# NeRF-3DTalker/NeRF-3DTalker-code

Hardware: AMD Instinct MI355X
Metric: rendered frames/sec @512^2 x 64 samples/ray (higher is better)
Workload: dtype bf16; 1 GPU; cfg2-R: 16 heads/GPU/step, 64x64 rays x 64 samples -> fused MLP+composite -> neural renderer -> 512x512 RGB (+ background image); rays_per_frame=4096, samples_per_ray=64, parallelism=frames sharded over 1 rank(s), no data-path collective, ranks_seen_by_backend=1

## Files before the change

### nerf-3dtalker-code_amd/csrc/nerf_fwd_x16.hip

```cpp
#include "x16_core.h"


#ifndef X16_SAVE_DEPTH
#define X16_SAVE_DEPTH 3
#endif
template <int PREC>
struct X16SaveStage {
    unsigned char* tile0;
    unsigned* gate0;
};

#define X16_BIAS_SLOT 1536
#ifndef X16_SAVE_LDS_BIAS
#define X16_SAVE_LDS_BIAS 1
#endif
struct X16BiasLds {
    unsigned char* slots;
    unsigned addr;
    __device__ __forceinline__ void stage_in(const float* table, const int n, const int slot, const int lane) const {
#pragma unroll
        for (int i = 0; i < 6; ++i)
            if (64 * i < n)
                __builtin_amdgcn_global_load_lds((const GLOBAL_AS void*)(table + 64 * i + lane), (LDS_AS void*)(slots + slot * X16_BIAS_SLOT + 256 * i), 4, 0, 0);
    }
};

template <int PREC, int NB, int WAVES, int KS, int KPE, int NT, int MODE, bool SAVE = false, class WS>
__device__ __forceinline__ void x16_stage(WS& ws, const float* __restrict__ bias,
                                          const typename X16<PREC>::frag (&pe_reg)[NB][4], const unsigned char* pe_lds,
                                          const typename X16<PREC>::frag (&hin)[NB][24], typename X16<PREC>::frag (&hout)[NB][24],
                                          float (&aux)[NB], float* const (&po)[NB], const bool (&live)[NB], const int lane,
                                          const X16SaveStage<PREC>* sv = nullptr, const short relu_lo = 0,
                                          const unsigned bias_lds = 0 ) {
    typedef typename X16<PREC>::frag frag;
    static_assert(!SAVE || NB == 1, "the training forward runs one block per wave");
    const int h = lane >> 5, c = lane & 31;
    float red[NB][32];
    unsigned gate_word = 0;
    const frag ones = X16<PREC>::ones_frag();
    float bias_cur = 0.0f, bias_nxt = 0.0f;
    constexpr bool LB = SAVE && X16_SAVE_LDS_BIAS;
    if constexpr (LB) {
        x16_bias_read<0>(bias_cur, bias_lds);
        asm volatile("s_waitcnt lgkmcnt(0)" : "+v"(bias_cur));
    } else {
        bias_cur = bias[c];
    }
    constexpr bool PACKS = (MODE == MODE_HIDDEN || MODE == MODE_LINEAR);
    f32x16 acc[1][NB];
    auto finish_half = [&](const int t, const int half) {
#pragma unroll
        for (int nb = 0; nb < NB; ++nb) {
            float v[8];
#pragma unroll
            for (int r = 0; r < 8; ++r) v[r] = acc[0][nb][8 * half + r];
            frag f = X16<PREC>::pack(v);
            if (MODE == MODE_HIDDEN) f = X16<PREC>::relu(f, relu_lo);
            hout[nb][2 * t + half] = f;
        }
    };
    static_for<0, NT>([&](auto ot_c) {
        constexpr int ot = decltype(ot_c)::value;
        constexpr int cur = 0;
        X16_T(const unsigned long long s0 = x16_now();)
        {
            const frag bf = X16<PREC>::bias_frag(bias_cur, h == 0);
            if constexpr (LB) {
                if constexpr (ot + 1 < NT) x16_bias_read<(ot + 1) * 128>(bias_nxt, bias_lds);
            } else {
                if (ot + 1 < NT) bias_cur = bias[(ot + 1) * 32 + c];
            }
            f32x16 zero;
#pragma unroll
            for (int r = 0; r < 16; ++r) zero[r] = 0.0f;
            const f32x16 binit = X16<PREC>::mfma(bf, ones, zero);
#pragma unroll
            for (int nb = 0; nb < NB; ++nb) acc[cur][nb] = binit;
        }
        X16_T(const unsigned long long s1 = x16_now(); const unsigned long long rv0 = ws.t_rv;)
        static_for<0, KS>([&](auto ks_c) {
            constexpr int ks = decltype(ks_c)::value;
            const frag a_cur = ws.template next<MODE == MODE_COMPOSITE, NT * KS, ot * KS + ks>();
#pragma unroll
            for (int nb = 0; nb < NB; ++nb) {
                frag b;
                if (ks < KPE) {
                    if (pe_lds) b = *reinterpret_cast<const frag*>(pe_lds + (nb * 4 + ks) * X16_PIECE);
                    else b = pe_reg[nb][ks < 4 ? ks : 0];
                } else {
                    b = hin[nb][ks >= KPE ? ks - KPE : 0];
                }
                acc[cur][nb] = X16<PREC>::mfma(a_cur, b, acc[cur][nb]);
            }
        });
        if constexpr (LB && ot + 1 < NT) {
            asm volatile("" : "+v"(bias_nxt), "+v"(acc[cur][0]));
            bias_cur = bias_nxt;
        }
        X16_T(const unsigned long long s2 = x16_now();)
        if (PACKS) {
            finish_half(ot, 0);
            finish_half(ot, 1);
        }
        if constexpr (SAVE && PACKS) {
#ifndef X16_DIAG_NOIMG
            x16_image_store<PREC>(hout[0][2 * ot], hout[0][2 * ot + 1], sv->tile0 + ot * 2 * X16_PIECE);
            ws.note_stores(2);
#endif
#ifndef X16_DIAG_NOGATE
            unsigned m = 0;
#pragma unroll
            for (int half = 0; half < 2; ++half) {
                const s16x8 hv = __builtin_bit_cast(s16x8, hout[0][2 * ot + half]);
#pragma unroll
                for (int j = 0; j < 8; ++j) m |= (hv[j] != 0 ? 1u : 0u) << (8 * half + j);
            }
            if constexpr (ot & 1) {
                __builtin_nontemporal_store(gate_word | (m << 16), sv->gate0 + (ot >> 1) * 64);
                ws.note_stores(1);
            } else {
                gate_word = m;
            }
#endif
        }
#pragma unroll
        for (int nb = 0; nb < NB; ++nb) {
            if (MODE == MODE_DENSITY) {
                aux[nb] = acc[cur][nb][0];
            } else if (MODE == MODE_COMPOSITE) {
#pragma unroll
                for (int r = 0; r < 16; ++r) red[nb][(ot & 1) * 16 + r] = fmaxf(acc[cur][nb][r], 0.0f) * aux[nb];
                if constexpr (SAVE) {
#pragma unroll
                    for (int half = 0; half < 2; ++half) {
                        float v[8];
#pragma unroll
                        for (int r = 0; r < 8; ++r) v[r] = fmaxf(acc[cur][nb][8 * half + r], 0.0f);
                        __builtin_nontemporal_store(X16<PREC>::pack(v), reinterpret_cast<frag*>(sv->tile0 + (2 * ot + half) * X16_PIECE));
                    }
                    ws.note_stores(2);
                }
                if (ot & 1) {
                    float s = butterfly32(red[nb], c);
                    const int v = ((c & 1) << 4) | ((c & 2) << 2) | (c & 4) | ((c & 8) >> 2) | ((c & 16) >> 4);
                    const int reg = v & 15, tile = (ot - 1) + (v >> 4);
                    if (live[nb]) po[nb][tile * 32 + (reg & 3) + 8 * (reg >> 2) + 4 * h] = s;
                }
            }
        }
        X16_T(const unsigned long long s3 = x16_now(); ws.t_bias += s1 - s0; ws.t_mfma += (s2 - s1) - (ws.t_rv - rv0); ws.t_epi += s3 - s2;
              if (ws.tl && ws.tile_no >= 20 && ws.tile_no < 34 && (threadIdx.x & 63) == 0) {
                  ws.tl[4 + 2 * (ws.tile_no - 20)] = (float)(s1 & 0xFFFFFF);
                  ws.tl[5 + 2 * (ws.tile_no - 20)] = (float)(s2 & 0xFFFFFF);
              }
              ++ws.tile_no;)
    });
}

struct X16TrainSave {
    unsigned char* xT;
    unsigned char* gS;
    float* geo;
    unsigned* gates;
};

template <int PREC, int NB, int WAVES, bool SAVE = false>
__device__ __forceinline__ void nerf_fwd_x16_body(
    const N3dtGeom& g, const unsigned char* __restrict__ packed, const float* __restrict__ fold, const float* __restrict__ xy,
    const float* __restrict__ R, const float* __restrict__ T, const float* __restrict__ Kinv, const float* __restrict__ t_rand,
    float* __restrict__ part, float* __restrict__ wlocal, int bpr, long total_blocks, unsigned char* lds, const int wave,
    const X16TrainSave tsv = X16TrainSave{nullptr, nullptr, nullptr, nullptr}) {
    typedef typename X16<PREC>::frag frag;
    const int lane = threadIdx.x & 63;
    const int c = lane & 31, h = lane >> 5;

    typedef WeightStream<PREC, WAVES, X16_NCHUNK, X16_NBUF, SAVE ? X16_SAVE_DEPTH : X16_DEPTH> WS;
    WS ws;
    ws.gsrc = packed + (size_t)wave * WS::PPW * X16_PIECE + lane * 16;
    ws.ring = lds;
    ws.lds_addr0 = (unsigned)(size_t)(LDS_AS unsigned char*)lds + lane * 16;
    ws.wave = wave;
    ws.prologue_issue();
    unsigned char* pe_lds = lds + X16_NBUF * X16_CH * X16_PIECE + (size_t)wave * NB * 4 * X16_PIECE + lane * 16;

    bool live[NB];
    float* po[NB];
    long blk[NB];
    float dist[NB], zval[NB];
    frag pe[NB][4];
    int frame = 0;
    long ray0 = 0;
#pragma unroll
    for (int nb = 0; nb < NB; ++nb) {
        long bidx = ((long)blockIdx.x * WAVES + wave) * NB + nb;
        live[nb] = bidx < total_blocks;
        if (!live[nb]) bidx = total_blocks - 1;
        blk[nb] = bidx;
        po[nb] = part + (size_t)bidx * N3DT_PART_STRIDE;
        const int sb = (int)(bidx % bpr);
        const long rayg = bidx / bpr;
        const int ray = (int)(rayg % g.n_rays);
        const int b = (int)(rayg / g.n_rays);
        if (nb == 0) frame = b, ray0 = rayg;
        float p[3];
        n3dt_sample_point(g, xy, R, T, Kinv, t_rand, b, ray, sb * X16_BS + c, p, dist[nb], zval[nb]);
        float rh[3], rl[3];
#pragma unroll
        for (int i = 0; i < 3; ++i) {
            const float inv2pi_hi = 0.15915494f, inv2pi_lo = 6.2195e-09f;
            rh[i] = p[i] * inv2pi_hi;
            rl[i] = fmaf(p[i], inv2pi_hi, -rh[i]) + p[i] * inv2pi_lo;
        }
#pragma unroll
        for (int ks = 0; ks < 4; ++ks) {
            float v[8];
#pragma unroll
            for (int j = 0; j < 8; ++j)
                v[j] = pe_fast(p[0], p[1], p[2], rh[0], rh[1], rh[2], rl[0], rl[1], rl[2],
                               32 * (ks >> 1) + 16 * (ks & 1) + 8 * (j >> 2) + 4 * h + (j & 3));
            pe[nb][ks] = X16<PREC>::pack(v);
            *reinterpret_cast<frag*>(pe_lds + (nb * 4 + ks) * X16_PIECE) = pe[nb][ks];
        }
    }
    const float* fb = fold + (size_t)__builtin_amdgcn_readfirstlane(frame) * N3DT_FOLD_STRIDE;
    const float* b10 = fb + n3dt_bias_offset(10);
#if defined(X16_DIAG_VD_SELECT_ALL)
#if defined(X16_DIAG_VD_TERNARY)
    b10 = g.vd_dim > 0 ? fold + n3dt_rayfold_offset(g.batch) + (size_t)__builtin_amdgcn_readfirstlane((int)ray0) * N3DT_RAYFOLD_STRIDE
                       : fb + n3dt_bias_offset(10);
#elif defined(X16_DIAG_VD_NO_RFL)
    if (g.vd_dim > 0) b10 = fold + n3dt_rayfold_offset(g.batch) + (size_t)ray0 * N3DT_RAYFOLD_STRIDE;
#else
    if (g.vd_dim > 0) b10 = fold + n3dt_rayfold_offset(g.batch) + (size_t)__builtin_amdgcn_readfirstlane((int)ray0) * N3DT_RAYFOLD_STRIDE;
#endif
#else
    if constexpr (NB == 1) {
        if (g.vd_dim > 0) b10 = fold + n3dt_rayfold_offset(g.batch) + (size_t)__builtin_amdgcn_readfirstlane((int)ray0) * N3DT_RAYFOLD_STRIDE;
    }
#endif
    X16SaveStage<PREC> svs;
    unsigned char* xT_blk = nullptr;
    const long rec = live[0] ? blk[0] : total_blocks;
    if constexpr (SAVE) {
        xT_blk = tsv.xT + (size_t)rec * X16_XT_TILES * 2 * X16_PIECE + x16_image_lane_offset(lane);
        x16_image_store<PREC>(pe[0][0], pe[0][1], xT_blk);
        x16_image_store<PREC>(pe[0][2], pe[0][3], xT_blk + 2 * X16_PIECE);
    }
    auto sv_hidden = [&](const int l) -> const X16SaveStage<PREC>* {
        if constexpr (SAVE) {
            svs.tile0 = xT_blk + (size_t)(2 + 12 * l) * 2 * X16_PIECE;
            svs.gate0 = tsv.gates + ((size_t)rec * 8 + l) * 6 * 64 + lane;
            return &svs;
        } else {
            return nullptr;
        }
    };
    X16BiasLds bl;
    if constexpr (SAVE && X16_SAVE_LDS_BIAS) {
        bl.slots = lds + X16_NBUF * X16_CH * X16_PIECE + (size_t)WAVES * NB * 4 * X16_PIECE + (size_t)wave * 2 * X16_BIAS_SLOT;
        bl.addr = (unsigned)(size_t)(LDS_AS unsigned char*)bl.slots + 4 * c;
        bl.stage_in(fb + n3dt_bias_offset(0), 384, 0, lane);
    }
    auto bias_slot = [&](const int k, const int next_table, const int next_n) -> unsigned {
        if constexpr (SAVE && X16_SAVE_LDS_BIAS) {
            if (next_table >= 0) bl.stage_in(next_table == 10 ? b10 : fb + n3dt_bias_offset(next_table), next_n, (k + 1) & 1, lane);
            return bl.addr + (k & 1) * X16_BIAS_SLOT;
        } else {
            return 0u;
        }
    };
    ws.prologue_wait();
    X16_T(if (wlocal && live[0]) ws.tl = wlocal + (size_t)blk[0] * X16_BS;)

    frag ha[NB][24], hb[NB][24];
    float aux[NB];
    x16_stage<PREC, NB, WAVES, 4, 4, 12, MODE_HIDDEN, SAVE>(ws, fb + n3dt_bias_offset(0), pe, nullptr, ha, ha, aux, po, live, lane, sv_hidden(0), 0, bias_slot(0, 1, 384));
    x16_stage<PREC, NB, WAVES, 24, 0, 12, MODE_HIDDEN, SAVE>(ws, fb + n3dt_bias_offset(1), pe, nullptr, ha, hb, aux, po, live, lane, sv_hidden(1), 0, bias_slot(1, 2, 384));
    x16_stage<PREC, NB, WAVES, 24, 0, 12, MODE_HIDDEN, SAVE>(ws, fb + n3dt_bias_offset(2), pe, nullptr, hb, ha, aux, po, live, lane, sv_hidden(2), 0, bias_slot(2, 3, 384));
    x16_stage<PREC, NB, WAVES, 24, 0, 12, MODE_HIDDEN, SAVE>(ws, fb + n3dt_bias_offset(3), pe, nullptr, ha, hb, aux, po, live, lane, sv_hidden(3), 0, bias_slot(3, 4, 384));
    x16_stage<PREC, NB, WAVES, 24, 0, 12, MODE_HIDDEN, SAVE>(ws, fb + n3dt_bias_offset(4), pe, nullptr, hb, ha, aux, po, live, lane, sv_hidden(4), 0, bias_slot(4, 5, 384));
    x16_stage<PREC, NB, WAVES, 28, 4, 12, MODE_HIDDEN, SAVE>(ws, fb + n3dt_bias_offset(5), pe, pe_lds, ha, hb, aux, po, live, lane, sv_hidden(5), 0, bias_slot(5, 6, 384));
    x16_stage<PREC, NB, WAVES, 24, 0, 12, MODE_HIDDEN, SAVE>(ws, fb + n3dt_bias_offset(6), pe, nullptr, hb, ha, aux, po, live, lane, sv_hidden(6), 0, bias_slot(6, 7, 384));
    x16_stage<PREC, NB, WAVES, 24, 0, 12, MODE_HIDDEN, SAVE>(ws, fb + n3dt_bias_offset(7), pe, nullptr, ha, hb, aux, po, live, lane, sv_hidden(7), 0, bias_slot(7, 10, 192));
    x16_stage<PREC, NB, WAVES, 24, 0, 1, MODE_DENSITY, false>(ws, fb + n3dt_bias_offset(8), pe, nullptr, hb, ha, aux, po, live, lane);
#pragma unroll
    for (int nb = 0; nb < NB; ++nb) {
        float sp = __shfl(aux[nb], c, 64);
        if constexpr (SAVE) {
            if (live[nb] && h == 0) {
                tsv.geo[(size_t)blk[nb] * 64 + c] = sp;
                tsv.geo[(size_t)blk[nb] * 64 + 32 + c] = dist[nb];
            }
        }
        float sigma = fmaxf(sp, 0.0f);
#if defined(X16_DIAG_REMASK_DEAD_LANES)
        asm volatile("" : "+v"(dist[nb]), "+v"(zval[nb]));
        if ((int)(blk[nb] % bpr) * X16_BS + c >= g.n_samples) dist[nb] = 0.0f, zval[nb] = 0.0f;
#endif
        float alpha = 1.0f - expf(-sigma * dist[nb]);
        float x = 1.0f - alpha + 1e-10f;
        float Tl = n3dt_exclusive_prod<32>(x, c);
        float w = alpha * Tl;
        float s0 = w, s1 = w * zval[nb];
#pragma unroll
        for (int off = 16; off > 0; off >>= 1) {
            s0 += __shfl_xor(s0, off, 32);
            s1 += __shfl_xor(s1, off, 32);
        }
        float tprod = __shfl(Tl * x, 31, 32);
        if (live[nb] && lane == 0) {
            po[nb][N3DT_G + 0] = s0;
            po[nb][N3DT_G + 1] = s1;
            po[nb][N3DT_G + 2] = tprod;
            po[nb][N3DT_G + 3] = 0.0f;
        }
#ifndef X16_STAMP
        if (live[nb] && wlocal && h == 0) wlocal[(size_t)blk[nb] * X16_BS + c] = w;
#endif
        aux[nb] = w;
    }
    if constexpr (SAVE) {
        svs.tile0 = tsv.gS + (size_t)rec * 12 * X16_PIECE + lane * 16;
        svs.gate0 = nullptr;
    }
    x16_stage<PREC, NB, WAVES, 24, 0, 6, MODE_COMPOSITE, SAVE>(ws, b10, pe, nullptr, hb, ha, aux, po, live, lane,
                                                                     SAVE ? &svs : nullptr, 0, bias_slot(8, -1, 0));
#ifdef X16_STAMP
    if (wlocal && lane == 0 && live[0]) {
        float* dbg = wlocal + (size_t)blk[0] * X16_BS;
        dbg[0] = (float)ws.t_bias;
        dbg[1] = (float)ws.t_mfma;
        dbg[2] = (float)ws.t_epi;
        dbg[3] = (float)ws.t_rv;
    }
#endif
}

template <int PREC, int NB, int WAVES>
__global__ __launch_bounds__(WAVES * 64, 1) void nerf_fwd_x16_kernel(
    N3dtGeom g, const unsigned char* __restrict__ packed, const float* __restrict__ fold, const float* __restrict__ xy,
    const float* __restrict__ R, const float* __restrict__ T, const float* __restrict__ Kinv, const float* __restrict__ t_rand,
    float* __restrict__ part, float* __restrict__ wlocal, int bpr, long total_blocks) {
    extern __shared__ __attribute__((aligned(16))) unsigned char lds[];
    const int wave = __builtin_amdgcn_readfirstlane(threadIdx.x >> 6);
    nerf_fwd_x16_body<PREC, NB, WAVES>(g, packed, fold, xy, R, T, Kinv, t_rand, part, wlocal, bpr, total_blocks, lds, wave);
}

template <int WAVES>
__global__ __launch_bounds__(WAVES * 64, 1) void nerf_fwd_x16_train_kernel(
    N3dtGeom g, const unsigned char* __restrict__ packed, const float* __restrict__ fold, const float* __restrict__ xy,
    const float* __restrict__ R, const float* __restrict__ T, const float* __restrict__ Kinv, const float* __restrict__ t_rand,
    float* __restrict__ part, float* __restrict__ wlocal, int bpr, long total_blocks, X16TrainSave tsv) {
    extern __shared__ __attribute__((aligned(16))) unsigned char lds[];
    const int wave = __builtin_amdgcn_readfirstlane(threadIdx.x >> 6);
    nerf_fwd_x16_body<N3DT_BF16, 1, WAVES, true>(g, packed, fold, xy, R, T, Kinv, t_rand, part, wlocal, bpr, total_blocks, lds, wave,
                                                        tsv);
}

#ifndef X16_TRAIN_WAVES
#define X16_TRAIN_WAVES 8
#endif
extern "C" void n3dt_launch_nerf_fwd_x16_train(const N3dtGeom* g, const void* packed, const float* fold, const float* xy, const float* R,
                                               const float* T, const float* Kinv, const float* t_rand, float* part, float* wlocal,
                                               void* xT, void* gS, float* geo, void* gates, hipStream_t stream) {
    constexpr int WAVES = X16_TRAIN_WAVES;
    const int bpr = (g->n_samples + X16_BS - 1) / X16_BS;
    const long total = (long)g->batch * g->n_rays * bpr;
    const int grid = (int)((total + WAVES - 1) / WAVES);
    const size_t lds_bytes = X16_NBUF * X16_CH * X16_PIECE + (size_t)WAVES * 4 * X16_PIECE + (size_t)WAVES * 2 * X16_BIAS_SLOT;
    auto kern = nerf_fwd_x16_train_kernel<WAVES>;
    (void)hipFuncSetAttribute(reinterpret_cast<const void*>(kern), hipFuncAttributeMaxDynamicSharedMemorySize, (int)lds_bytes);
    X16TrainSave tsv{reinterpret_cast<unsigned char*>(xT), reinterpret_cast<unsigned char*>(gS), geo, reinterpret_cast<unsigned*>(gates)};
    hipLaunchKernelGGL(kern, dim3(grid), dim3(WAVES * 64), lds_bytes, stream, *g, reinterpret_cast<const unsigned char*>(packed), fold, xy,
                       R, T, Kinv, t_rand, part, wlocal, bpr, total, tsv);
}

template <int PREC, int NB, int WAVES>
static void launch_x16(const N3dtGeom* g, const void* packed, const float* fold, const float* xy, const float* R, const float* T,
                       const float* Kinv, const float* t_rand, float* part, float* wlocal, hipStream_t stream) {
    const int bpr = (g->n_samples + X16_BS - 1) / X16_BS;
    const long total = (long)g->batch * g->n_rays * bpr;
    const long per_wg = (long)WAVES * NB;
    const int grid = (int)((total + per_wg - 1) / per_wg);
    const size_t lds_bytes = X16_NBUF * X16_CH * X16_PIECE + (size_t)WAVES * NB * 4 * X16_PIECE;
    auto kern = nerf_fwd_x16_kernel<PREC, NB, WAVES>;
    (void)hipFuncSetAttribute(reinterpret_cast<const void*>(kern), hipFuncAttributeMaxDynamicSharedMemorySize, (int)lds_bytes);
    hipLaunchKernelGGL(kern, dim3(grid), dim3(WAVES * 64), lds_bytes, stream, *g, reinterpret_cast<const unsigned char*>(packed),
                       fold, xy, R, T, Kinv, t_rand, part, wlocal, bpr, total);
}

extern "C" void n3dt_launch_nerf_fwd_x16(const N3dtGeom* g, int precision, const void* packed, const float* fold, const float* xy,
                                         const float* R, const float* T, const float* Kinv, const float* t_rand, float* part,
                                         float* wlocal, hipStream_t stream) {
    static const int wide = [] {
        const char* e = getenv("N3DT_X16_TILING");
        const char* d = getenv("N3DT_X16_TILING2_DIAG");
        const int t = e ? atoi(e) : X16_DEFAULT_TILING;
        return (t == 2 && !(d && atoi(d) == 1)) ? 1 : t;
    }();
    const long blocks = (long)g->batch * g->n_rays * ((g->n_samples + X16_BS - 1) / X16_BS);
    const bool use_wide = wide == 2 && g->vd_dim == 0 && (((long)g->n_rays * ((g->n_samples + X16_BS - 1) / X16_BS)) % 2 == 0) && blocks >= 2;
    if (precision == N3DT_BF16) {
        if (use_wide) launch_x16<N3DT_BF16, 2, 4>(g, packed, fold, xy, R, T, Kinv, t_rand, part, wlocal, stream);
        else launch_x16<N3DT_BF16, 1, 8>(g, packed, fold, xy, R, T, Kinv, t_rand, part, wlocal, stream);
    } else {
        if (use_wide) launch_x16<N3DT_F16, 2, 4>(g, packed, fold, xy, R, T, Kinv, t_rand, part, wlocal, stream);
        else launch_x16<N3DT_F16, 1, 8>(g, packed, fold, xy, R, T, Kinv, t_rand, part, wlocal, stream);
    }
}
```

### nerf-3dtalker-code_amd/csrc/x16_core.h

```cpp
#pragma once
#include <stdlib.h>

#include <type_traits>

#include "n3dt_device.h"
#include "n3dt_layout.h"

typedef __bf16 bf16x8 __attribute__((ext_vector_type(8)));

#define X16_BS 32
#define X16_CH 24
#define X16_PIECE 1024
#define X16_NCHUNK (2280 / X16_CH)
#define X16_XT_TILES 98
#define GLOBAL_AS __attribute__((address_space(1)))
#define LDS_AS __attribute__((address_space(3)))

template <int PREC>
struct X16;
template <>
struct X16<N3DT_BF16> {
    typedef bf16x8 frag;
    static __device__ __forceinline__ f32x16 mfma(frag a, frag b, f32x16 c) {
        return __builtin_amdgcn_mfma_f32_32x32x16_bf16(a, b, c, 0, 0, 0);
    }
    static __device__ __forceinline__ f32x4 mfma16(frag a, frag b, f32x4 c) {
        return __builtin_amdgcn_mfma_f32_16x16x32_bf16(a, b, c, 0, 0, 0);
    }
    static __device__ __forceinline__ frag pack(const float* v) {
        frag f;
#pragma unroll
        for (int j = 0; j < 8; ++j) f[j] = (__bf16)v[j];
        return f;
    }
    static __device__ __forceinline__ frag relu(frag f, short lo) {
        s16x8 s = __builtin_bit_cast(s16x8, f);
        s = __builtin_elementwise_max(s, (s16x8)(lo));
        return __builtin_bit_cast(frag, s);
    }
    static __device__ __forceinline__ frag bias_frag(float b, bool lower_half) {
        __bf16 hi = (__bf16)b;
        __bf16 lo = (__bf16)(b - (float)hi);
        frag f;
#pragma unroll
        for (int j = 0; j < 8; ++j) f[j] = (__bf16)0.0f;
        if (lower_half) {
            f[0] = hi;
            f[1] = lo;
        }
        return f;
    }
    static __device__ __forceinline__ frag ones_frag() {
        frag f;
#pragma unroll
        for (int j = 0; j < 8; ++j) f[j] = (__bf16)(j < 2 ? 1.0f : 0.0f);
        return f;
    }
};
template <>
struct X16<N3DT_F16> {
    typedef f16x8 frag;
    static __device__ __forceinline__ f32x16 mfma(frag a, frag b, f32x16 c) {
        return __builtin_amdgcn_mfma_f32_32x32x16_f16(a, b, c, 0, 0, 0);
    }
    static __device__ __forceinline__ f32x4 mfma16(frag a, frag b, f32x4 c) {
        return __builtin_amdgcn_mfma_f32_16x16x32_f16(a, b, c, 0, 0, 0);
    }
    static __device__ __forceinline__ frag pack(const float* v) {
        frag f;
#pragma unroll
        for (int j = 0; j < 8; ++j) f[j] = (_Float16)v[j];
        return f;
    }
    static __device__ __forceinline__ frag relu(frag f, short lo) {
        s16x8 s = __builtin_bit_cast(s16x8, f);
        s = __builtin_elementwise_max(s, (s16x8)(lo));
        return __builtin_bit_cast(frag, s);
    }
    static __device__ __forceinline__ frag bias_frag(float b, bool lower_half) {
        _Float16 hi = (_Float16)b;
        _Float16 lo = (_Float16)(b - (float)hi);
        frag f;
#pragma unroll
        for (int j = 0; j < 8; ++j) f[j] = (_Float16)0.0f;
        if (lower_half) {
            f[0] = hi;
            f[1] = lo;
        }
        return f;
    }
    static __device__ __forceinline__ frag ones_frag() {
        frag f;
#pragma unroll
        for (int j = 0; j < 8; ++j) f[j] = (_Float16)(j < 2 ? 1.0f : 0.0f);
        return f;
    }
};

#ifndef X16_DEPTH
#define X16_DEPTH 3
#endif
#ifndef X16_DEFAULT_TILING
#define X16_DEFAULT_TILING 1
#endif
#ifndef X16_NBUF
#define X16_NBUF 3
#endif
#define X16_CHUNK_BYTES (X16_CH * X16_PIECE)

#ifdef X16_STAMP
__device__ __forceinline__ unsigned long long x16_now() {
    unsigned long long t;
    __builtin_amdgcn_sched_barrier(0);
    asm volatile("s_memtime %0\n\ts_waitcnt lgkmcnt(0)" : "=s"(t)::"memory");
    __builtin_amdgcn_sched_barrier(0);
    return t;
}
#define X16_T(x) x
#else
#define X16_T(x)
#endif

template <int I, int N, class F>
__device__ __forceinline__ void static_for(F&& f) {
    if constexpr (I < N) {
        f(std::integral_constant<int, I>{});
        static_for<I + 1, N>(f);
    }
}

template <class T>
__device__ __forceinline__ void x16_pin(T& v) {
    static_assert(sizeof(T) <= 8, "scalar register pair at most");
    asm volatile("" : "+s"(v));
}
template <class T>
__device__ __forceinline__ void x16_pin(T*& p) {
    unsigned long long v = (unsigned long long)p;
    asm volatile("" : "+s"(v));
    p = (T*)(GLOBAL_AS T*)v;
}
template <class T>
__device__ __forceinline__ void x16_pin_v(T*& p) {
    unsigned long long v = (unsigned long long)p;
    asm volatile("" : "+v"(v));
    p = (T*)(GLOBAL_AS T*)v;
}

#ifndef X16_RV_RAW
#define X16_RV_RAW 0
#endif
#ifndef X16_NT_STORE
#define X16_NT_STORE 1
#endif
template <int PREC, int WAVES, int NCHUNK = X16_NCHUNK, int NBUF = X16_NBUF, int DEPTH = X16_DEPTH>
struct WeightStream {
    X16_T(unsigned long long t_rv = 0; unsigned long long t_mfma = 0; unsigned long long t_epi = 0; unsigned long long t_bias = 0;
          int tile_no = 0; float* tl = nullptr;)
    typedef typename X16<PREC>::frag frag;
    const unsigned char* gsrc;
    unsigned char* ring;
    unsigned lds_addr0;
    unsigned cur_addr, nxt_addr;
    int chunk;
    int meets;
    int wave;
    int limit;
    int src_c;
    frag a[DEPTH];
    static constexpr int PPW = X16_CH / WAVES;

    __device__ __forceinline__ void issue(int c) {
        const unsigned char* src = gsrc + (size_t)src_c * X16_CHUNK_BYTES;
        src_c = src_c + 1 == NCHUNK ? 0 : src_c + 1;
        unsigned char* dst = ring + (c % NBUF) * X16_CHUNK_BYTES + wave * PPW * X16_PIECE;
#pragma unroll
        for (int i = 0; i < PPW; ++i)
            __builtin_amdgcn_global_load_lds((const GLOBAL_AS void*)(src + i * X16_PIECE), (LDS_AS void*)(dst + i * X16_PIECE), 16, 0,
                                             0);
    }
    __device__ __forceinline__ void prologue_issue(const int passes = 1) {
        limit = passes * NCHUNK;
        src_c = 0;
#pragma unroll
        for (int i = 0; i < NBUF - 1; ++i)
            if (i < limit) issue(i);
    }
    __device__ __forceinline__ void drain() { asm volatile("s_waitcnt vmcnt(0) lgkmcnt(0)" ::: "memory"); }
    __device__ __forceinline__ void prologue_wait() {
        asm volatile("s_waitcnt vmcnt(0) lgkmcnt(0)" ::: "memory");
        __syncthreads();
        chunk = 0;
        meets = 0;
        vm_cur = 0;
        vm_prev = 0;
        cur_addr = lds_addr0;
        nxt_addr = lds_addr0 + X16_CHUNK_BYTES;
        preload<0>();
    }
    template <int J>
    __device__ __forceinline__ void preload() {
        if constexpr (J < DEPTH - 1) {
            read_frag<J * X16_PIECE>(a[J], cur_addr);
            preload<J + 1>();
        }
    }
    int vm_cur = 0, vm_prev = 0;
    __device__ __forceinline__ void note_stores(const int n) { vm_cur += n; }
    template <int K>
    __device__ __forceinline__ static void wait_vm() {
        asm volatile("s_waitcnt vmcnt(%0)" ::"i"(K) : "memory");
    }
    __device__ __forceinline__ void rendezvous() {
        int newer = limit - 2 - meets;
        newer = newer < 0 ? 0 : (newer > NBUF - 3 ? NBUF - 3 : newer);
        int k = newer * PPW + vm_cur + (NBUF > 3 ? vm_prev : 0);
        if (k > 15) k = 15;
        static_for<0, 16>([&](auto k_c) {
            constexpr int K = decltype(k_c)::value;
            if (k == K) wait_vm<K>();
        });
#if X16_RV_RAW
        __builtin_amdgcn_s_barrier();
        asm volatile("" ::: "memory");
#else
        __syncthreads();
#endif
#ifndef X16_NODMA
        if (meets + NBUF - 1 < limit) issue(meets + NBUF - 1);
#endif
        vm_prev = vm_cur;
        vm_cur = 0;
        ++meets;
    }
    template <int OFF>
    __device__ __forceinline__ void read_frag(frag& dst, const unsigned addr) {
        asm volatile("ds_read_b128 %0, %1 offset:%2" : "=v"(dst) : "v"(addr), "i"(OFF) : "memory");
    }
    template <int YOUNGER = DEPTH - 1>
    __device__ __forceinline__ void await_frag(frag& f) {
        asm volatile("s_waitcnt lgkmcnt(%1)" : "+v"(f) : "i"(YOUNGER));
    }
    template <bool LAST, int NP, int P>
    __device__ __forceinline__ frag next() {
        constexpr int rv = X16_CH - DEPTH;
        if (P % X16_CH == rv) {
            X16_T(const unsigned long long r0 = x16_now();)
            rendezvous();
            X16_T(t_rv += x16_now() - r0;)
        }
        constexpr int Q = P + DEPTH - 1;
#ifdef X16_NOLDS
        if ((P + 1) % X16_CH == 0) ++chunk;
        return a[0];
#endif
        if (!(LAST && Q >= NP)) {
            const unsigned addr = (Q % X16_CH < P % X16_CH) ? nxt_addr : cur_addr;
            read_frag<(Q % X16_CH) * X16_PIECE>(a[Q % DEPTH], addr);
        }
        constexpr int younger = (LAST && NP - 1 - P < DEPTH - 1) ? NP - 1 - P : DEPTH - 1;
        await_frag<younger>(a[P % DEPTH]);
        const frag r = a[P % DEPTH];
        if ((P + 1) % X16_CH == 0) {
            ++chunk;
            cur_addr = nxt_addr;
            nxt_addr = lds_addr0 + ((chunk + 1) % NBUF) * X16_CHUNK_BYTES;
        }
        return r;
    }
    __device__ __forceinline__ void settle() {
        asm volatile("s_waitcnt lgkmcnt(0)" : "+v"(a[0]));
#pragma unroll
        for (int i = 1; i < DEPTH; ++i) asm volatile("" : "+v"(a[i]));
    }
};

__device__ __forceinline__ float x16_lrelu02(const float a) {
    const float b = 0.2f * a;
    float r;
    asm("v_max_f32 %0, %1, %2" : "=v"(r) : "v"(a), "v"(b));
    return r;
}

template <int OFF>
__device__ __forceinline__ void x16_bias_read(float& dst, const unsigned addr) {
    asm volatile("ds_read_b32 %0, %1 offset:%2" : "=v"(dst) : "v"(addr), "i"(OFF) : "memory");
}

__device__ __forceinline__ float pick3(const int d, const float a, const float b, const float c) {
    const float ab = d == 0 ? a : b;
    return d == 2 ? c : ab;
}
__device__ __forceinline__ float pe_fast(const float p0, const float p1, const float p2, const float h0, const float h1,
                                         const float h2, const float l0, const float l1, const float l2, const int ch) {
    const int cc = ch < 3 ? 0 : ch - 3;
    const int k = cc / 6, w = cc % 6, dim = w >= 3 ? w - 3 : w;
    const float sc = (float)(1 << k);
    const float hi = pick3(dim, h0, h1, h2), lo = pick3(dim, l0, l1, l2);
    const float r = __builtin_amdgcn_fractf(hi * sc) + lo * sc + (w >= 3 ? 0.25f : 0.0f);
    const float sv = __builtin_amdgcn_sinf(r);
    const float raw = pick3(ch, p0, p1, p2);
    return ch < 3 ? raw : (ch >= N3DT_PE_DIM ? 0.0f : sv);
}

enum { MODE_HIDDEN = 0, MODE_LINEAR = 1, MODE_DENSITY = 2, MODE_COMPOSITE = 3 };


__device__ __forceinline__ float butterfly32(float (&v)[32], const int c) {
#pragma unroll
    for (int step = 0; step < 5; ++step) {
        const int m = 16 >> step;
        const bool bit = (c & m) != 0;
        const int n = 32 >> step;
#pragma unroll
        for (int i = 0; i < n / 2; ++i) {
            float keep = bit ? v[2 * i + 1] : v[2 * i];
            float send = bit ? v[2 * i] : v[2 * i + 1];
            v[i] = keep + __shfl_xor(send, m, 64);
        }
    }
    return v[0];
}

__device__ __forceinline__ int x16_image_lane_offset(const int lane) { return 64 * (lane & 31) + 16 * (lane >> 5); }
template <int PREC>
__device__ __forceinline__ void x16_image_store(const typename X16<PREC>::frag f0, const typename X16<PREC>::frag f1, unsigned char* dst) {
    typedef typename X16<PREC>::frag frag;
#if X16_NT_STORE
    __builtin_nontemporal_store(f0, reinterpret_cast<frag*>(dst));
    __builtin_nontemporal_store(f1, reinterpret_cast<frag*>(dst + 32));
#else
    *reinterpret_cast<frag*>(dst) = f0;
    *reinterpret_cast<frag*>(dst + 32) = f1;
#endif
}
__device__ __forceinline__ unsigned x16_tr_lane_offset(const int lane) {
    const int r = lane & 31, h = lane >> 5, q = (r & 15) >> 2, p = r & 3;
    return 64u * (8 * h + q) + 32u * (r >> 4) + 8u * ((p & 1) * 2 + (p >> 1));
}
__device__ __forceinline__ unsigned x16_tr_lane_offset_natural(const int lane) {
    const int r = lane & 31, h = lane >> 5, q = (r & 15) >> 2, p = r & 3;
    return 64u * (8 * h + q) + 32u * (r >> 4) + 8u * p;
}
typedef unsigned x16_u32x2 __attribute__((ext_vector_type(2)));
typedef unsigned x16_u32x4 __attribute__((ext_vector_type(4)));
template <int OFF>
__device__ __forceinline__ void x16_tr_issue(x16_u32x2& d, const unsigned lds_addr) {
    asm volatile("ds_read_b64_tr_b16 %0, %1 offset:%2" : "=v"(d) : "v"(lds_addr), "i"(OFF) : "memory");
}
struct X16TrTile {
    x16_u32x2 q[4];
    template <int TILE_OFF>
    __device__ __forceinline__ void issue(const unsigned tile_lane) {
        x16_tr_issue<TILE_OFF>(q[0], tile_lane);
        x16_tr_issue<TILE_OFF + 256>(q[1], tile_lane);
        x16_tr_issue<TILE_OFF + 1024>(q[2], tile_lane);
        x16_tr_issue<TILE_OFF + 1280>(q[3], tile_lane);
    }
    __device__ __forceinline__ void pin() {
#pragma unroll
        for (int i = 0; i < 4; ++i) asm volatile("" : "+v"(q[i]));
    }
    __device__ __forceinline__ bf16x8 frag(const int sp) const {
        const x16_u32x4 v = {q[2 * sp][0], q[2 * sp][1], q[2 * sp + 1][0], q[2 * sp + 1][1]};
        return __builtin_bit_cast(bf16x8, v);
    }
};
__device__ __forceinline__ void x16_tr_settle() { asm volatile("s_waitcnt lgkmcnt(0)" ::: "memory"); }
```

Before: 1969 frames/s.

## Stage biases in LDS for inference path and load accumulator bias directly

Biases are now staged into per-wave LDS slots for the NB==1 inference forward as well, not only the training save path. The accumulator is initialised straight from ds_read_b128 bias vectors, so the bias-via-MFMA (bias frag times ones) is dropped. An alternative form adds the bias after the k-loop with packed adds. The lgkmcnt waits in the fragment pipeline are widened to account for the extra in-flight bias reads. This removes one MFMA and per-lane global bias loads per output tile, at the cost of more LDS per workgroup and tighter waitcnt bookkeeping.

```diff
diff --git a/nerf-3dtalker-code_amd/csrc/nerf_fwd_x16.hip b/nerf-3dtalker-code_amd/csrc/nerf_fwd_x16.hip
--- a/nerf-3dtalker-code_amd/csrc/nerf_fwd_x16.hip
+++ b/nerf-3dtalker-code_amd/csrc/nerf_fwd_x16.hip
@@ -10,42 +10,39 @@
     unsigned* gate0;
 };
 
+#ifndef X16_BIAS_FORM
+#define X16_BIAS_FORM 1
+#endif
 #define X16_BIAS_SLOT 1536
-#ifndef X16_SAVE_LDS_BIAS
-#define X16_SAVE_LDS_BIAS 1
-#endif
 struct X16BiasLds {
     unsigned char* slots;
     unsigned addr;
-    __device__ __forceinline__ void stage_in(const float* table, const int n, const int slot, const int lane) const {
+    __device__ __forceinline__ void stage_in(const float* table, const int n, const int slot, const int lane, const int off = 0) const {
 #pragma unroll
         for (int i = 0; i < 6; ++i)
             if (64 * i < n)
-                __builtin_amdgcn_global_load_lds((const GLOBAL_AS void*)(table + 64 * i + lane), (LDS_AS void*)(slots + slot * X16_BIAS_SLOT + 256 * i), 4, 0, 0);
+                __builtin_amdgcn_global_load_lds((const GLOBAL_AS void*)(table + 64 * i + lane),
+                                                 (LDS_AS void*)(slots + slot * X16_BIAS_SLOT + off + 256 * i), 4, 0, 0);
     }
 };
 
 template <int PREC, int NB, int WAVES, int KS, int KPE, int NT, int MODE, bool SAVE = false, class WS>
-__device__ __forceinline__ void x16_stage(WS& ws, const float* __restrict__ bias,
+__device__ __forceinline__ void x16_stage(WS& ws, const unsigned bias_lds , const float* bias_g,
                                           const typename X16<PREC>::frag (&pe_reg)[NB][4], const unsigned char* pe_lds,
                                           const typename X16<PREC>::frag (&hin)[NB][24], typename X16<PREC>::frag (&hout)[NB][24],
                                           float (&aux)[NB], float* const (&po)[NB], const bool (&live)[NB], const int lane,
-                                          const X16SaveStage<PREC>* sv = nullptr, const short relu_lo = 0,
-                                          const unsigned bias_lds = 0 ) {
+                                          const X16SaveStage<PREC>* sv = nullptr, const short relu_lo = 0) {
     typedef typename X16<PREC>::frag frag;
     static_assert(!SAVE || NB == 1, "the training forward runs one block per wave");
     const int h = lane >> 5, c = lane & 31;
     float red[NB][32];
     unsigned gate_word = 0;
-    const frag ones = X16<PREC>::ones_frag();
-    float bias_cur = 0.0f, bias_nxt = 0.0f;
-    constexpr bool LB = SAVE && X16_SAVE_LDS_BIAS;
-    if constexpr (LB) {
-        x16_bias_read<0>(bias_cur, bias_lds);
-        asm volatile("s_waitcnt lgkmcnt(0)" : "+v"(bias_cur));
-    } else {
-        bias_cur = bias[c];
-    }
+    constexpr int DEPTH = WS::depth;
+    constexpr int KB = KS - 1 - DEPTH;
+    static_assert(KB >= 0, "a stage needs DEPTH + 1 k-steps per tile");
+    constexpr int FORM = NB > 1 ? 2 : (SAVE ? 1 : X16_BIAS_FORM);
+    float bias_cur = 0.0f;
+    if constexpr (FORM == 2) bias_cur = bias_g[c];
     constexpr bool PACKS = (MODE == MODE_HIDDEN || MODE == MODE_LINEAR);
     f32x16 acc[1][NB];
     auto finish_half = [&](const int t, const int half) {
@@ -63,24 +60,31 @@
         constexpr int ot = decltype(ot_c)::value;
         constexpr int cur = 0;
         X16_T(const unsigned long long s0 = x16_now();)
-        {
+        f32x4 bq[4];
+        if constexpr (FORM == 1) x16_bias_read4<ot * 128>(bq, bias_lds);
+        if constexpr (FORM == 2) {
             const frag bf = X16<PREC>::bias_frag(bias_cur, h == 0);
-            if constexpr (LB) {
-                if constexpr (ot + 1 < NT) x16_bias_read<(ot + 1) * 128>(bias_nxt, bias_lds);
-            } else {
-                if (ot + 1 < NT) bias_cur = bias[(ot + 1) * 32 + c];
-            }
+            if (ot + 1 < NT) bias_cur = bias_g[(ot + 1) * 32 + c];
             f32x16 zero;
 #pragma unroll
             for (int r = 0; r < 16; ++r) zero[r] = 0.0f;
-            const f32x16 binit = X16<PREC>::mfma(bf, ones, zero);
+            const f32x16 binit = X16<PREC>::mfma(bf, X16<PREC>::ones_frag(), zero);
 #pragma unroll
             for (int nb = 0; nb < NB; ++nb) acc[cur][nb] = binit;
         }
         X16_T(const unsigned long long s1 = x16_now(); const unsigned long long rv0 = ws.t_rv;)
         static_for<0, KS>([&](auto ks_c) {
             constexpr int ks = decltype(ks_c)::value;
-            const frag a_cur = ws.template next<MODE == MODE_COMPOSITE, NT * KS, ot * KS + ks>();
+            constexpr int xtra = FORM == 1 ? (ks < DEPTH - 1 ? 4 : 0) : FORM == 0 ? (ks > KB && ks < KB + DEPTH ? 4 : 0) : 0;
+            const frag a_cur = ws.template next<MODE == MODE_COMPOSITE, NT * KS, ot * KS + ks, xtra>();
+            if constexpr (FORM == 0 && ks == KB) x16_bias_read4<ot * 128>(bq, bias_lds);
+            if constexpr (FORM == 1 && ks == 0) {
+                asm volatile("s_waitcnt lgkmcnt(1)" : "+v"(bq[0]), "+v"(bq[1]), "+v"(bq[2]), "+v"(bq[3]));
+#pragma unroll
+                for (int nb = 0; nb < NB; ++nb)
+#pragma unroll
+                    for (int r = 0; r < 16; ++r) acc[cur][nb][r] = bq[r >> 2][r & 3];
+            }
 #pragma unroll
             for (int nb = 0; nb < NB; ++nb) {
                 frag b;
@@ -90,12 +94,20 @@
                 } else {
                     b = hin[nb][ks >= KPE ? ks - KPE : 0];
                 }
-                acc[cur][nb] = X16<PREC>::mfma(a_cur, b, acc[cur][nb]);
+                if (FORM == 0 && ks == 0) {
+                    f32x16 zero;
+#pragma unroll
+                    for (int r = 0; r < 16; ++r) zero[r] = 0.0f;
+                    acc[cur][nb] = X16<PREC>::mfma(a_cur, b, zero);
+                } else {
+                    acc[cur][nb] = X16<PREC>::mfma(a_cur, b, acc[cur][nb]);
+                }
             }
         });
-        if constexpr (LB && ot + 1 < NT) {
-            asm volatile("" : "+v"(bias_nxt), "+v"(acc[cur][0]));
-            bias_cur = bias_nxt;
+        if constexpr (FORM == 0) {
+            asm volatile("" : "+v"(bq[0]), "+v"(bq[1]), "+v"(bq[2]), "+v"(bq[3]), "+v"(acc[cur][0]));
+#pragma unroll
+            for (int nb = 0; nb < NB; ++nb) x16_add_bias(acc[cur][nb], bq);
         }
         X16_T(const unsigned long long s2 = x16_now();)
         if (PACKS) {
@@ -256,33 +268,33 @@
         }
     };
     X16BiasLds bl;
-    if constexpr (SAVE && X16_SAVE_LDS_BIAS) {
-        bl.slots = lds + X16_NBUF * X16_CH * X16_PIECE + (size_t)WAVES * NB * 4 * X16_PIECE + (size_t)wave * 2 * X16_BIAS_SLOT;
-        bl.addr = (unsigned)(size_t)(LDS_AS unsigned char*)bl.slots + 4 * c;
-        bl.stage_in(fb + n3dt_bias_offset(0), 384, 0, lane);
-    }
-    auto bias_slot = [&](const int k, const int next_table, const int next_n) -> unsigned {
-        if constexpr (SAVE && X16_SAVE_LDS_BIAS) {
-            if (next_table >= 0) bl.stage_in(next_table == 10 ? b10 : fb + n3dt_bias_offset(next_table), next_n, (k + 1) & 1, lane);
-            return bl.addr + (k & 1) * X16_BIAS_SLOT;
+    bl.slots = lds + X16_NBUF * X16_CH * X16_PIECE + (size_t)WAVES * NB * 4 * X16_PIECE + (size_t)wave * 2 * X16_BIAS_SLOT;
+    bl.addr = (unsigned)(size_t)(LDS_AS unsigned char*)bl.slots + 16 * h;
+    if constexpr (NB == 1) bl.stage_in(fb + n3dt_bias_offset(0), 384, 0, lane);
+    auto bias_slot = [&](const int k) -> unsigned {
+        if (NB > 1) {
+        } else if (k < 7) {
+            bl.stage_in(fb + n3dt_bias_offset(k + 1), 384, (k + 1) & 1, lane);
         } else {
-            return 0u;
-        }
+            bl.stage_in(fb + n3dt_bias_offset(8), 64, 0, lane);
+            bl.stage_in(b10, 192, 0, lane, 256);
+        }
+        return bl.addr + (k & 1) * X16_BIAS_SLOT;
     };
     ws.prologue_wait();
     X16_T(if (wlocal && live[0]) ws.tl = wlocal + (size_t)blk[0] * X16_BS;)
 
     frag ha[NB][24], hb[NB][24];
     float aux[NB];
-    x16_stage<PREC, NB, WAVES, 4, 4, 12, MODE_HIDDEN, SAVE>(ws, fb + n3dt_bias_offset(0), pe, nullptr, ha, ha, aux, po, live, lane, sv_hidden(0), 0, bias_slot(0, 1, 384));
-    x16_stage<PREC, NB, WAVES, 24, 0, 12, MODE_HIDDEN, SAVE>(ws, fb + n3dt_bias_offset(1), pe, nullptr, ha, hb, aux, po, live, lane, sv_hidden(1), 0, bias_slot(1, 2, 384));
-    x16_stage<PREC, NB, WAVES, 24, 0, 12, MODE_HIDDEN, SAVE>(ws, fb + n3dt_bias_offset(2), pe, nullptr, hb, ha, aux, po, live, lane, sv_hidden(2), 0, bias_slot(2, 3, 384));
-    x16_stage<PREC, NB, WAVES, 24, 0, 12, MODE_HIDDEN, SAVE>(ws, fb + n3dt_bias_offset(3), pe, nullptr, ha, hb, aux, po, live, lane, sv_hidden(3), 0, bias_slot(3, 4, 384));
-    x16_stage<PREC, NB, WAVES, 24, 0, 12, MODE_HIDDEN, SAVE>(ws, fb + n3dt_bias_offset(4), pe, nullptr, hb, ha, aux, po, live, lane, sv_hidden(4), 0, bias_slot(4, 5, 384));
-    x16_stage<PREC, NB, WAVES, 28, 4, 12, MODE_HIDDEN, SAVE>(ws, fb + n3dt_bias_offset(5), pe, pe_lds, ha, hb, aux, po, live, lane, sv_hidden(5), 0, bias_slot(5, 6, 384));
-    x16_stage<PREC, NB, WAVES, 24, 0, 12, MODE_HIDDEN, SAVE>(ws, fb + n3dt_bias_offset(6), pe, nullptr, hb, ha, aux, po, live, lane, sv_hidden(6), 0, bias_slot(6, 7, 384));
-    x16_stage<PREC, NB, WAVES, 24, 0, 12, MODE_HIDDEN, SAVE>(ws, fb + n3dt_bias_offset(7), pe, nullptr, ha, hb, aux, po, live, lane, sv_hidden(7), 0, bias_slot(7, 10, 192));
-    x16_stage<PREC, NB, WAVES, 24, 0, 1, MODE_DENSITY, false>(ws, fb + n3dt_bias_offset(8), pe, nullptr, hb, ha, aux, po, live, lane);
+    x16_stage<PREC, NB, WAVES, 4, 4, 12, MODE_HIDDEN, SAVE>(ws, bias_slot(0), fb + n3dt_bias_offset(0), pe, nullptr, ha, ha, aux, po, live, lane, sv_hidden(0));
+    x16_stage<PREC, NB, WAVES, 24, 0, 12, MODE_HIDDEN, SAVE>(ws, bias_slot(1), fb + n3dt_bias_offset(1), pe, nullptr, ha, hb, aux, po, live, lane, sv_hidden(1));
+    x16_stage<PREC, NB, WAVES, 24, 0, 12, MODE_HIDDEN, SAVE>(ws, bias_slot(2), fb + n3dt_bias_offset(2), pe, nullptr, hb, ha, aux, po, live, lane, sv_hidden(2));
+    x16_stage<PREC, NB, WAVES, 24, 0, 12, MODE_HIDDEN, SAVE>(ws, bias_slot(3), fb + n3dt_bias_offset(3), pe, nullptr, ha, hb, aux, po, live, lane, sv_hidden(3));
+    x16_stage<PREC, NB, WAVES, 24, 0, 12, MODE_HIDDEN, SAVE>(ws, bias_slot(4), fb + n3dt_bias_offset(4), pe, nullptr, hb, ha, aux, po, live, lane, sv_hidden(4));
+    x16_stage<PREC, NB, WAVES, 28, 4, 12, MODE_HIDDEN, SAVE>(ws, bias_slot(5), fb + n3dt_bias_offset(5), pe, pe_lds, ha, hb, aux, po, live, lane, sv_hidden(5));
+    x16_stage<PREC, NB, WAVES, 24, 0, 12, MODE_HIDDEN, SAVE>(ws, bias_slot(6), fb + n3dt_bias_offset(6), pe, nullptr, hb, ha, aux, po, live, lane, sv_hidden(6));
+    x16_stage<PREC, NB, WAVES, 24, 0, 12, MODE_HIDDEN, SAVE>(ws, bias_slot(7), fb + n3dt_bias_offset(7), pe, nullptr, ha, hb, aux, po, live, lane, sv_hidden(7));
+    x16_stage<PREC, NB, WAVES, 24, 0, 1, MODE_DENSITY, false>(ws, bl.addr, fb + n3dt_bias_offset(8), pe, nullptr, hb, ha, aux, po, live, lane);
 #pragma unroll
     for (int nb = 0; nb < NB; ++nb) {
         float sp = __shfl(aux[nb], c, 64);
@@ -323,8 +335,8 @@
         svs.tile0 = tsv.gS + (size_t)rec * 12 * X16_PIECE + lane * 16;
         svs.gate0 = nullptr;
     }
-    x16_stage<PREC, NB, WAVES, 24, 0, 6, MODE_COMPOSITE, SAVE>(ws, b10, pe, nullptr, hb, ha, aux, po, live, lane,
-                                                                     SAVE ? &svs : nullptr, 0, bias_slot(8, -1, 0));
+    x16_stage<PREC, NB, WAVES, 24, 0, 6, MODE_COMPOSITE, SAVE>(ws, bl.addr + 256, b10, pe, nullptr, hb, ha, aux, po, live, lane,
+                                                                     SAVE ? &svs : nullptr);
 #ifdef X16_STAMP
     if (wlocal && lane == 0 && live[0]) {
         float* dbg = wlocal + (size_t)blk[0] * X16_BS;
@@ -382,7 +394,7 @@
     const long total = (long)g->batch * g->n_rays * bpr;
     const long per_wg = (long)WAVES * NB;
     const int grid = (int)((total + per_wg - 1) / per_wg);
-    const size_t lds_bytes = X16_NBUF * X16_CH * X16_PIECE + (size_t)WAVES * NB * 4 * X16_PIECE;
+    const size_t lds_bytes = X16_NBUF * X16_CH * X16_PIECE + (size_t)WAVES * NB * 4 * X16_PIECE + (NB == 1 ? (size_t)WAVES * 2 * X16_BIAS_SLOT : 0);
     auto kern = nerf_fwd_x16_kernel<PREC, NB, WAVES>;
     (void)hipFuncSetAttribute(reinterpret_cast<const void*>(kern), hipFuncAttributeMaxDynamicSharedMemorySize, (int)lds_bytes);
     hipLaunchKernelGGL(kern, dim3(grid), dim3(WAVES * 64), lds_bytes, stream, *g, reinterpret_cast<const unsigned char*>(packed),
diff --git a/nerf-3dtalker-code_amd/csrc/x16_core.h b/nerf-3dtalker-code_amd/csrc/x16_core.h
--- a/nerf-3dtalker-code_amd/csrc/x16_core.h
+++ b/nerf-3dtalker-code_amd/csrc/x16_core.h
@@ -169,6 +169,7 @@
     int src_c;
     frag a[DEPTH];
     static constexpr int PPW = X16_CH / WAVES;
+    static constexpr int depth = DEPTH;
 
     __device__ __forceinline__ void issue(int c) {
         const unsigned char* src = gsrc + (size_t)src_c * X16_CHUNK_BYTES;
@@ -241,7 +242,7 @@
     __device__ __forceinline__ void await_frag(frag& f) {
         asm volatile("s_waitcnt lgkmcnt(%1)" : "+v"(f) : "i"(YOUNGER));
     }
-    template <bool LAST, int NP, int P>
+    template <bool LAST, int NP, int P, int XTRA = 0>
     __device__ __forceinline__ frag next() {
         constexpr int rv = X16_CH - DEPTH;
         if (P % X16_CH == rv) {
@@ -259,7 +260,8 @@
             read_frag<(Q % X16_CH) * X16_PIECE>(a[Q % DEPTH], addr);
         }
         constexpr int younger = (LAST && NP - 1 - P < DEPTH - 1) ? NP - 1 - P : DEPTH - 1;
-        await_frag<younger>(a[P % DEPTH]);
+        static_assert(younger + XTRA <= 15, "lgkmcnt is a 4-bit count");
+        await_frag<younger + XTRA>(a[P % DEPTH]);
         const frag r = a[P % DEPTH];
         if ((P + 1) % X16_CH == 0) {
             ++chunk;
@@ -285,6 +287,25 @@
 template <int OFF>
 __device__ __forceinline__ void x16_bias_read(float& dst, const unsigned addr) {
     asm volatile("ds_read_b32 %0, %1 offset:%2" : "=v"(dst) : "v"(addr), "i"(OFF) : "memory");
+}
+template <int OFF>
+__device__ __forceinline__ void x16_bias_read4(f32x4 (&dst)[4], const unsigned addr) {
+    asm volatile("ds_read_b128 %0, %1 offset:%2" : "=v"(dst[0]) : "v"(addr), "i"(OFF) : "memory");
+    asm volatile("ds_read_b128 %0, %1 offset:%2" : "=v"(dst[1]) : "v"(addr), "i"(OFF + 32) : "memory");
+    asm volatile("ds_read_b128 %0, %1 offset:%2" : "=v"(dst[2]) : "v"(addr), "i"(OFF + 64) : "memory");
+    asm volatile("ds_read_b128 %0, %1 offset:%2" : "=v"(dst[3]) : "v"(addr), "i"(OFF + 96) : "memory");
+}
+
+typedef float x16_f32x2 __attribute__((ext_vector_type(2)));
+__device__ __forceinline__ void x16_add_bias(f32x16& acc, const f32x4 (&bq)[4]) {
+#pragma unroll
+    for (int p = 0; p < 8; ++p) {
+        x16_f32x2 a = {acc[2 * p], acc[2 * p + 1]};
+        const x16_f32x2 b = {bq[p >> 1][2 * (p & 1)], bq[p >> 1][2 * (p & 1) + 1]};
+        asm("v_pk_add_f32 %0, %1, %2" : "=v"(a) : "v"(a), "v"(b));
+        acc[2 * p] = a[0];
+        acc[2 * p + 1] = a[1];
+    }
 }
 
 __device__ __forceinline__ float pick3(const int d, const float a, const float b, const float c) {
```

Result: no change. 1984 frames/s (median of 6 runs) (+0.8%).
